# neuripss2020/kccotgan

Measured on AMD Instinct MI355X. Metric: sinkhorn_loss_evals_per_sec, higher is better.
Workload: dtype f32; 1 GPU; BASELINE configs[1]: Moving-MNIST shape B=64,T=30,64x64x1, J=8, 100 Sinkhorn iters, compute_sinkhorn_loss fwd+bwd; global_batch=64, parallelism=single GPU, sinkhorn_exact_shortcut=off, launch=hipGraph replay of forward+backward

## Files before the change

kccotgan_amd/csrc/sinkhorn.hip:

```cpp
#include "common.h"
#include <math.h>
#include "options.h"

#pragma clang fp contract(off)

namespace kccot {

constexpr int SK_MAXN = 128;
constexpr int SK_FUSED_MAXPROB = 4;
constexpr int SK_MAXT = 1024;
constexpr float LOG2E = 1.4426950408889634f;
constexpr float LN2 = 0.6931471805599453f;

__device__ __forceinline__ float fast_exp(float x) { return __builtin_amdgcn_exp2f(x * LOG2E); }
__device__ __forceinline__ float fast_log(float x) { return __builtin_amdgcn_logf(x) * LN2; }

#ifdef KCCOT_DIAG
#ifndef KCCOT_DIAG_IT
#define KCCOT_DIAG_IT 50
#endif
#define KCCOT_DIAG_SLOTS 32
#define KCCOT_STAMP(SLOT) KCCOT_STAMP_IF(it == KCCOT_DIAG_IT, SLOT)
#define KCCOT_STAMP_IF(COND, SLOT)                                                                \
    do {                                                                                          \
        if (a.diag && (COND)) {                                                                   \
            unsigned long long tt_;                                                               \
            __builtin_amdgcn_sched_barrier(0);                                                    \
            asm volatile("s_memtime %0\n\ts_waitcnt lgkmcnt(0)" : "=s"(tt_)::"memory");          \
            __builtin_amdgcn_sched_barrier(0);                                                    \
            if ((threadIdx.x & 63) == 0) a.diag[(blockIdx.x * 16 + (threadIdx.x >> 6)) * KCCOT_DIAG_SLOTS + (SLOT)] = tt_; \
        }                                                                                         \
    } while (0)
#define KCCOT_STAMP_DRAINED(SLOT)                                                                 \
    do {                                                                                          \
        if (a.diag) asm volatile("s_waitcnt vmcnt(0)" ::: "memory");                              \
        KCCOT_STAMP_IF(true, SLOT);                                                               \
    } while (0)
#else
#define KCCOT_STAMP(SLOT) do {} while (0)
#define KCCOT_STAMP_IF(COND, SLOT) do {} while (0)
#define KCCOT_STAMP_DRAINED(SLOT) do {} while (0)
#endif

struct SinkArgs {
    const float* C;
    int n, L, Lmin, stop_mode;
    float eps, inv_eps, thresh;
    float* u_hist;
    float* v_hist;
    float* cost_out;
    int32_t* nits_out;
    float* pi_out;
    unsigned long long* diag;
    float* loss_out;
    int* ticket;
    int shortcut;
    const float* wa;
    const float* wb;
    int w_div;
};

__device__ __forceinline__ const float* weights_of(const float* wa, const float* wb, int w_div, int p, int n, bool rows) {
    if (w_div == 2) return wa + (int64_t)(p / 3) * n;
    if (w_div) return rows ? (p == 2 ? wb : wa) : (p == 1 ? wa : wb);
    return (rows ? wa : wb) + (int64_t)p * n;
}
__device__ __forceinline__ bool weight_ok(float w) { return w > 0.f && w < INFINITY; }

template <int EPT>
__device__ __forceinline__ void load_other(float (&o)[EPT], const float* arr, int q) {
    if constexpr (EPT >= 4) {
#pragma unroll
        for (int m = 0; m < EPT; m += 4) {
            const float4 v = *reinterpret_cast<const float4*>(arr + q * EPT + m);
            o[m] = v.x; o[m + 1] = v.y; o[m + 2] = v.z; o[m + 3] = v.w;
        }
    } else {
#pragma unroll
        for (int m = 0; m < EPT; ++m) o[m] = arr[q * EPT + m];
    }
}

typedef float f32x2 __attribute__((ext_vector_type(2)));

template <int N>
__device__ __forceinline__ void keep_in_regs(float (&r)[N]) {
    if constexpr (N >= 2) {
#pragma unroll
        for (int m = 0; m < N; m += 2) {
            f32x2 t = {r[m], r[m + 1]};
            asm volatile("" : "+v"(t));
            r[m] = t.x; r[m + 1] = t.y;
        }
    } else {
        asm volatile("" : "+v"(r[0]));
    }
}

template <int EPT, int LPR, bool ROW>
__device__ __forceinline__ float half_step(const float (&c2)[EPT], float self, const float* other, int q, float lw2) {
    float o[EPT];
    load_other<EPT>(o, other, q);
    float y[EPT];
    if constexpr (EPT >= 2) {
#pragma unroll
        for (int m = 0; m < EPT; m += 2) {
            f32x2 cc = {c2[m], c2[m + 1]}, oo = {o[m], o[m + 1]}, ss = {self, self};
            const f32x2 t = ROW ? ((ss - cc) + oo) : ((oo - cc) + ss);
            y[m] = t.x; y[m + 1] = t.y;
        }
    } else {
        y[0] = ROW ? ((self - c2[0]) + o[0]) : ((o[0] - c2[0]) + self);
    }
    float mx = y[0];
#pragma unroll
    for (int m = 1; m < EPT; ++m) mx = fmaxf(mx, y[m]);
    mx = seg_max<LPR>(mx);
    const float shift = (mx > -INFINITY && mx < INFINITY) ? mx : 0.f;
    float e[EPT];
    if constexpr (EPT >= 2) {
        const f32x2 sh = {shift, shift};
#pragma unroll
        for (int m = 0; m < EPT; m += 2) {
            const f32x2 yy = {y[m], y[m + 1]};
            const f32x2 d = yy - sh;
            e[m] = __builtin_amdgcn_exp2f(d.x);
            e[m + 1] = __builtin_amdgcn_exp2f(d.y);
        }
    } else {
        e[0] = __builtin_amdgcn_exp2f(y[0] - shift);
    }
#pragma unroll
    for (int w = 1; w < EPT; w *= 2)
#pragma unroll
        for (int m = 0; m + w < EPT; m += 2 * w) e[m] += e[m + w];
    const float s = seg_sum<LPR>(e[0]);
    const float lse2 = __builtin_amdgcn_logf(s) + shift;
    return (lw2 - lse2) + self;
}

template <int EPT, int LPR>
__device__ __forceinline__ void load_costs(const float* __restrict__ C, int n, int line, int q, float k2,
                                           float (&crow)[EPT], float (&ccol)[EPT]) {
#pragma unroll
    for (int m = 0; m < EPT; ++m) {
        const int idx = q * EPT + m;
        const bool ok = line < n && idx < n;
        crow[m] = ok ? C[(int64_t)line * n + idx] * k2 : INFINITY;
        ccol[m] = ok ? C[(int64_t)idx * n + line] * k2 : INFINITY;
    }
}


__device__ __forceinline__ void shortcut_mismatch(int& bits, float sn, float cur, float p2, float p3, float p4) {
    const unsigned b = __float_as_uint(sn);
    bits |= (b != __float_as_uint(cur) ? 2 : 0) | (b != __float_as_uint(p2) ? 4 : 0) |
           (b != __float_as_uint(p3) ? 8 : 0) | (b != __float_as_uint(p4) ? 16 : 0);
}
__device__ __forceinline__ void shortcut_vote(int bits, bool active, int t, int* mis, int it) {
    if (!active) bits = 0;
    int wb = 0;
#pragma unroll
    for (int pp = 1; pp <= 4; ++pp)
        if (__builtin_amdgcn_ballot_w64((bits >> pp) & 1)) wb |= 1 << pp;
    if ((t & 63) == 0 && wb) atomicOr(&mis[it & 3], wb);
}
__device__ __forceinline__ int shortcut_period(int* mis, int it, int t, int& mprev) {
    const int mcur = mis[it & 3];
    if (t == 0) mis[(it + 2) & 3] = 0;
    int per = 0;
#pragma unroll
    for (int pp = 4; pp >= 1; --pp)
        if (it - 1 >= pp && !((mprev >> pp) & 1)) per = pp;
    mprev = mcur;
    return per;
}
__device__ __forceinline__ int shortcut_resume(int L, int Lmin, int stop_mode) {
    int first_stop = (stop_mode == KCCOT_STOP_INDEX) ? Lmin + 1 : Lmin;
    if (first_stop < 1) first_stop = 1;
    return (L < first_stop ? L : first_stop) - 1;
}
__device__ __forceinline__ void fill_history_rows(float* hu, float* hv, int NS, int n, int t, int nits, int K1, int per) {
    const int lo = nits - per + 1;
    for (int e = t; e < (K1 - nits) * n; e += blockDim.x) {
        const int k = nits + 1 + e / n, i = e % n;
        const int src = lo + (k - lo) % per;
        hu[k * NS + i] = hu[src * NS + i];
        hv[k * NS + i] = hv[src * NS + i];
    }
}

template <int EPT>
__device__ __forceinline__ float cost_partial(const float (&crow)[EPT], const float (&craw)[EPT], float ui, const float* v,
                                              int n, int q, bool active) {
    float ov[EPT];
    load_other<EPT>(ov, v, q);
    float part = 0.f;
#pragma unroll
    for (int m = 0; m < EPT; ++m) {
        const float pi = __builtin_amdgcn_exp2f((ui - crow[m]) + ov[m]);
        const float sum = part + pi * craw[m];
        part = (active && q * EPT + m < n) ? sum : part;
    }
    return part;
}
template <int EPT, bool ROW>
__device__ __forceinline__ void load_costs_raw(const float* C, int n, int line, int q, float k2, float (&c2)[EPT],
                                               float (&craw)[EPT]) {
#pragma unroll
    for (int m = 0; m < EPT; ++m) {
        const int idx = q * EPT + m;
        const bool ok = line < n && idx < n;
        craw[m] = ok ? C[ROW ? (int64_t)line * n + idx : (int64_t)idx * n + line] : 0.f;
        c2[m] = ok ? craw[m] * k2 : INFINITY;
    }
}
template <int EPT, bool ROW>
__device__ __forceinline__ void load_costs_raw(const float* C, int n, int line, int q, float k2, float (&c2)[EPT]) {
    float craw[EPT];
    load_costs_raw<EPT, ROW>(C, n, line, q, k2, c2, craw);
}

__device__ __forceinline__ float cost_of_waves(const float* red, int nw) {
    float v[16];
#pragma unroll
    for (int w = 0; w < 16; ++w) v[w] = red[w];
    float r = 0.f;
#pragma unroll
    for (int w = 0; w < 16; ++w) r = w < nw ? r + v[w] : r;
    return r;
}

template <int NPROB>
__device__ __forceinline__ void publish_cost(float* const& cost_out, int32_t* const& nits_out, float* const& loss_out,
                                             int* const& ticket, int p, float cost, int nits, int computed, const float* w,
                                             bool combine) {
    __hip_atomic_store(cost_out + p, cost, __ATOMIC_RELAXED, __HIP_MEMORY_SCOPE_AGENT);
    nits_out[p] = nits;
    nits_out[gridDim.x + p] = computed;
    if (!combine) return;
    asm volatile("s_waitcnt vmcnt(0)" ::: "memory");
    const int tk = __hip_atomic_fetch_add(ticket, 1, __ATOMIC_RELAXED, __HIP_MEMORY_SCOPE_AGENT);
    if (tk == (int)gridDim.x - 1) {
        float c[NPROB];
        if constexpr (NPROB == 3) {
#pragma unroll
            for (int pp = 0; pp < 3; ++pp) c[pp] = __hip_atomic_load(cost_out + pp, __ATOMIC_RELAXED, __HIP_MEMORY_SCOPE_AGENT);
        } else {
            float o[3];
#pragma unroll
            for (int k = 0; k < 3; ++k)
                o[k] = __hip_atomic_load(cost_out + ((p + 1 + k) & 3), __ATOMIC_RELAXED, __HIP_MEMORY_SCOPE_AGENT);
#pragma unroll
            for (int pp = 0; pp < 4; ++pp) {
                const int k = (pp - p - 1) & 3;
                c[pp] = k == 0 ? o[0] : k == 1 ? o[1] : k == 2 ? o[2] : cost;
            }
        }
        float l = w[0] * c[0];
#pragma unroll
        for (int pp = 1; pp < NPROB; ++pp) l += w[pp] * c[pp];
        loss_out[0] = l;
        __hip_atomic_store(ticket, 0, __ATOMIC_RELAXED, __HIP_MEMORY_SCOPE_AGENT);
    }
}

template <bool ROW>
__device__ __forceinline__ void final_cost_adjoint(float c2, float self, float other, bool ok, float g, float& d, float& ss) {
    const float cc = ok ? c2 : 0.f;
    const float pv = ok ? __builtin_amdgcn_exp2f(ROW ? ((self - cc) + other) : ((other - cc) + self)) : 0.f;
    d = ROW ? g * pv * (1.f - cc * LN2) : 0.f;
    ss += pv * cc;
}

template <int EPT>
__device__ __forceinline__ void park_dc_cols(float* tile, const float (&dcol)[EPT], int n, int line, int q, bool active) {
    if (active) {
#pragma unroll
        for (int m = 0; m < EPT; ++m) {
            const int idx = q * EPT + m;
            if (idx < n) tile[idx * (n + 1) + line] = dcol[m];
        }
    }
}
template <int EPT>
__device__ __forceinline__ void take_dc_cols(const float* tile, float (&drow)[EPT], int n, int line, int q, bool active) {
#pragma unroll
    for (int m = 0; m < EPT; ++m) {
        const int idx = q * EPT + m;
        drow[m] += tile[(active && idx < n) ? line * (n + 1) + idx : 0];
    }
}
template <int EPT>
__device__ __forceinline__ void store_dc_rows(float* dC, const float (&drow)[EPT], int n, int line, int q, bool active) {
    if (active) {
#pragma unroll
        for (int m = 0; m < EPT; ++m) {
            const int idx = q * EPT + m;
            if (idx < n) dC[(int64_t)line * n + idx] = drow[m];
        }
    }
}

template <int EPT, int LPR, bool SHORTCUT, bool WEIGHTED>
__device__ __forceinline__ void sinkhorn_fwd_body(const SinkArgs& a) {
    __shared__ __attribute__((aligned(16))) float u_s[SK_MAXN + 16 * 16];
    __shared__ __attribute__((aligned(16))) float v_s[SK_MAXN + 16 * 16];
    __shared__ float red[16];
    const int p = blockIdx.x, n = a.n;
    const int t = threadIdx.x, line = t / LPR, q = t % LPR;
    const bool active = line < n;
    int pc = p;
    if constexpr (WEIGHTED) { if (a.w_div == 2) pc = p % 3; }
    const float* C = a.C + (int64_t)pc * n * n;
    const float k2 = a.inv_eps * LOG2E;

    float crow[EPT], ccol[EPT];
    load_costs<EPT, LPR>(C, n, line, q, k2, crow, ccol);
    for (int i = t; i < SK_MAXN + 16 * 16; i += blockDim.x) { u_s[i] = 0.f; v_s[i] = 0.f; }
    __syncthreads();

    const float lw2 = __builtin_amdgcn_logf(1.0f / (float)n);
    float lwu = lw2, lwv = lw2;
    bool bad = false;
    if constexpr (WEIGHTED) {
        const float wu = active ? weights_of(a.wa, a.wb, a.w_div, p, n, true)[line] : 1.f;
        const float wv = active ? weights_of(a.wa, a.wb, a.w_div, p, n, false)[line] : 1.f;
        bad = __syncthreads_or(!(weight_ok(wu) && weight_ok(wv)));
        lwu = __builtin_amdgcn_logf(wu);
        lwv = __builtin_amdgcn_logf(wv);
    }
    const int Lrun = (WEIGHTED && bad) ? 0 : a.L;
    const float err_scale = a.eps * LN2;

    __shared__ float ring_u[4][SK_MAXN], ring_v[4][SK_MAXN];
    __shared__ int mis[4];
    if (SHORTCUT) {
        if (t < 4) mis[t] = 0;
        __syncthreads();
    }
    bool detect = SHORTCUT;
    int computed = 0;
    int mprev = ~0;
    float pu2 = 0.f, pu3 = 0.f, pu4 = 0.f, pv2 = 0.f, pv3 = 0.f, pv4 = 0.f;

    int nits = 0;
    float ui = 0.f, vj = 0.f;
    for (int it = 0; it < Lrun; ++it) {
        KCCOT_STAMP(0);
        const float un = half_step<EPT, LPR, true>(crow, ui, v_s, q, lwu);
        KCCOT_STAMP(1);
        const float du = (active && q == 0) ? fabsf(un - ui) : 0.f;
        int bits = 0;
        if (SHORTCUT && detect) {
            shortcut_mismatch(bits, un, ui, pu2, pu3, pu4);
            pu4 = pu3; pu3 = pu2; pu2 = ui;
        }
        ui = un;
        if (active && q == 0) {
            u_s[line] = un;
            if (a.u_hist) a.u_hist[((int64_t)p * a.L + it) * n + line] = un;
            if (SHORTCUT && detect) ring_u[it & 3][line] = un;
        }
        KCCOT_STAMP(2);
        lds_barrier();
        KCCOT_STAMP(3);
        const float vn = half_step<EPT, LPR, false>(ccol, vj, u_s, q, lwv);
        KCCOT_STAMP(4);
        if (SHORTCUT && detect) {
            shortcut_mismatch(bits, vn, vj, pv2, pv3, pv4);
            pv4 = pv3; pv3 = pv2; pv2 = vj;
            shortcut_vote(bits, active, t, mis, it);
        }
        vj = vn;
        if (active && q == 0) {
            v_s[line] = vn;
            if (a.v_hist) a.v_hist[((int64_t)p * a.L + it) * n + line] = vn;
            if (SHORTCUT && detect) ring_v[it & 3][line] = vn;
        }
        KCCOT_STAMP(5);
        lds_barrier();
        KCCOT_STAMP(6);
        nits = it + 1;
        ++computed;
        const bool reached = (a.stop_mode == KCCOT_STOP_INDEX) ? (it >= a.Lmin) : (nits >= a.Lmin);
        if (reached && it + 1 < a.L) {
            const float err = block_sum(du, red) * err_scale;
            if (a.thresh > err) break;
        }
        if (SHORTCUT && detect) {
            const int per = shortcut_period(mis, it, t, mprev);
            KCCOT_STAMP(7);
            if (per) {
                detect = false;
                const int K1 = shortcut_resume(a.L, a.Lmin, a.stop_mode);
                if (K1 > nits) {
                    const int lo = nits - per + 1;
                    if (a.u_hist) {
                        for (int e = t; e < (K1 - nits) * n; e += blockDim.x) {
                            const int k = nits + 1 + e / n, i = e % n;
                            const int slot = (lo + (k - lo) % per - 1) & 3;
                            a.u_hist[((int64_t)p * a.L + (k - 1)) * n + i] = ring_u[slot][i];
                            a.v_hist[((int64_t)p * a.L + (k - 1)) * n + i] = ring_v[slot][i];
                        }
                    }
                    const int slot = (lo + (K1 - lo) % per - 1) & 3;
                    if (t < n) { u_s[t] = ring_u[slot][t]; v_s[t] = ring_v[slot][t]; }
                    __syncthreads();
                    ui = u_s[active ? line : 0];
                    vj = v_s[active ? line : 0];
                    nits = K1;
                    it = K1 - 1;
                }
            }
        }
    }

    float part = 0.f;
    if (active) {
#pragma unroll
        for (int m = 0; m < EPT; ++m) {
            const int idx = q * EPT + m;
            if (idx < n) {
                float pi = __builtin_amdgcn_exp2f((ui - crow[m]) + v_s[idx]);
                if (WEIGHTED && bad) pi = NAN;
                part += pi * C[(int64_t)line * n + idx];
                if (a.pi_out) a.pi_out[(int64_t)p * n * n + (int64_t)line * n + idx] = pi;
            }
        }
    }
    float cost = block_sum(part, red);
    if (WEIGHTED && bad) { cost = NAN; nits = -1; }
    if (t == 0) {
        const float w[3] = {2.0f, -1.0f, -1.0f};
        publish_cost<3>(a.cost_out, a.nits_out, a.loss_out, a.ticket, p, cost, nits, computed, w, a.loss_out != nullptr);
    }
}

template <int EPT, int LPR>
__global__ __launch_bounds__(SK_MAXT) void sinkhorn_fwd_reg(SinkArgs a) { sinkhorn_fwd_body<EPT, LPR, true, false>(a); }
template <int EPT, int LPR>
__global__ __launch_bounds__(SK_MAXT) void sinkhorn_fwd_reg_full(SinkArgs a) { sinkhorn_fwd_body<EPT, LPR, false, false>(a); }
template <int EPT, int LPR>
__global__ __launch_bounds__(SK_MAXT) void sinkhorn_fwd_reg_w(SinkArgs a) { sinkhorn_fwd_body<EPT, LPR, true, true>(a); }
template <int EPT, int LPR>
__global__ __launch_bounds__(SK_MAXT) void sinkhorn_fwd_reg_full_w(SinkArgs a) { sinkhorn_fwd_body<EPT, LPR, false, true>(a); }

struct SinkBwdArgs {
    const float* C;
    const float* u_hist;
    const float* v_hist;
    const int32_t* nits;
    const float* gcost;
    float* dC;
    int n, L;
    float eps, inv_eps;
    int div_weights;
    const float* wa;
    const float* wb;
    int w_div;
    float* da;
    float* db;
};

template <int EPT, int LPR, bool WEIGHTED, bool DW = false>
__device__ __forceinline__ void sinkhorn_bwd_body(const SinkBwdArgs& a) {
    static_assert(WEIGHTED || !DW, "the weight gradient belongs to the weighted sweep");
    constexpr int PADN = SK_MAXN + 16 * 16;
    __shared__ __attribute__((aligned(16))) float Ua[WEIGHTED ? 2 : 1][WEIGHTED ? PADN : 4];
    __shared__ __attribute__((aligned(16))) float Va[WEIGHTED ? 2 : 1][WEIGHTED ? PADN : 4];
    __shared__ float lab[WEIGHTED ? 2 : 1][WEIGHTED ? SK_MAXN : 1];
    __shared__ __attribute__((aligned(16))) float U[2][PADN];
    __shared__ __attribute__((aligned(16))) float V[2][PADN];
    __shared__ __attribute__((aligned(16))) float gu[PADN];
    __shared__ __attribute__((aligned(16))) float gv[PADN];
    __shared__ double sab[DW ? 2 : 1][DW ? SK_MAXN : 1];
    __shared__ float gvf[DW ? SK_MAXN : 1];
    __shared__ double mode[DW ? 2 : 1];
    const int p = blockIdx.x, n = a.n;
    const int t = threadIdx.x, line = t / LPR, q = t % LPR;
    const bool active = line < n;
    int pc = p;
    if constexpr (WEIGHTED) { if (a.w_div == 2) pc = p % 3; }
    const float* C = a.C + (int64_t)pc * n * n;
    const float k2 = a.inv_eps * LOG2E;
    const float g = a.div_weights ? (p == 0 ? 2.0f : -1.0f) * a.gcost[0] : a.gcost[p];
    const int nits = a.nits[p];
    const float* uh = a.u_hist + (int64_t)p * a.L * n;
    const float* vh = a.v_hist + (int64_t)p * a.L * n;
    if constexpr (WEIGHTED) {
        if (nits < 0) {
            if (active) {
#pragma unroll
                for (int m = 0; m < EPT; ++m) {
                    const int idx = q * EPT + m;
                    if (idx < n) a.dC[(int64_t)p * n * n + (int64_t)line * n + idx] = NAN;
                }
                if constexpr (DW) {
                    if (q == 0) { a.da[(int64_t)p * n + line] = NAN; a.db[(int64_t)p * n + line] = NAN; }
                }
            }
            return;
        }
        if (t < n) {
            lab[0][t] = __builtin_amdgcn_logf(weights_of(a.wa, a.wb, a.w_div, p, n, true)[t]);
            lab[1][t] = __builtin_amdgcn_logf(weights_of(a.wa, a.wb, a.w_div, p, n, false)[t]);
        }
    }

    float crow[EPT], ccol[EPT], drow[EPT], dcol[EPT];
    load_costs<EPT, LPR>(C, n, line, q, k2, crow, ccol);
#pragma unroll
    for (int m = 0; m < EPT; ++m) { drow[m] = 0.f; dcol[m] = 0.f; }
    for (int i = t; i < PADN; i += blockDim.x) {
        U[0][i] = U[1][i] = V[0][i] = V[1][i] = 0.f;
        gu[i] = gv[i] = 0.f;
        if constexpr (WEIGHTED) Ua[0][i] = Ua[1][i] = Va[0][i] = Va[1][i] = 0.f;
    }
    if constexpr (DW) { if (t < SK_MAXN) sab[0][t] = sab[1][t] = 0.0; }
    __syncthreads();
    auto hist_u = [&](int it, int i) { return it >= 1 ? uh[(int64_t)(it - 1) * n + i] : 0.f; };
    auto hist_v = [&](int it, int i) { return it >= 1 ? vh[(int64_t)(it - 1) * n + i] : 0.f; };
    if (t < n) {
        U[nits & 1][t] = hist_u(nits, t);
        V[nits & 1][t] = hist_v(nits, t);
        V[(nits - 1) & 1][t] = hist_v(nits - 1, t);
        if constexpr (WEIGHTED) {
            Ua[nits & 1][t] = hist_u(nits, t) - lab[0][t];
            Va[nits & 1][t] = hist_v(nits, t) - lab[1][t];
            Va[(nits - 1) & 1][t] = hist_v(nits - 1, t) - lab[1][t];
        }
    }
    float nu = (t < n) ? hist_u(nits - 1, t) : 0.f;
    float nv = (t < n) ? hist_v(nits - 2, t) : 0.f;
    __syncthreads();

    const int lsafe = active ? line : 0;
    {
        const float* Uc = U[nits & 1];
        const float* Vc = V[nits & 1];
        const float ui = Uc[lsafe], vj = Vc[lsafe];
        float ov[EPT], ou[EPT];
        load_other<EPT>(ov, Vc, q);
        load_other<EPT>(ou, Uc, q);
        float su = 0.f, sv = 0.f;
#pragma unroll
        for (int m = 0; m < EPT; ++m) {
            const bool ok = active && (q * EPT + m) < n;
            const float cr = ok ? crow[m] : 0.f, cc = ok ? ccol[m] : 0.f;
            const float pr = ok ? __builtin_amdgcn_exp2f((ui - cr) + ov[m]) : 0.f;
            drow[m] = g * pr * (1.f - cr * LN2);
            su += pr * cr;
            const float pc = ok ? __builtin_amdgcn_exp2f((ou[m] - cc) + vj) : 0.f;
            sv += pc * cc;
        }
        su = seg_sum<LPR>(su);
        sv = seg_sum<LPR>(sv);
        if (active && q == 0) {
            const float gvn = g * sv * LN2;
            gu[line] = g * su * LN2; gv[line] = gvn;
            if constexpr (DW) gvf[line] = nits > 0 ? gvn : 0.f;
        }
    }
    const float lw2 = __builtin_amdgcn_logf(1.0f / (float)n);
    __syncthreads();

    for (int it = nits; it >= 1; --it) {
        const float* Uc = U[it & 1];
        const float* Vc = V[it & 1];
        const float* Vp = V[(it - 1) & 1];
        {
            const float ui = WEIGHTED ? Uc[lsafe] : Uc[lsafe] - lw2;
            float ov[EPT], og[EPT];
            load_other<EPT>(ov, WEIGHTED ? Va[it & 1] : Vc, q);
            load_other<EPT>(og, gv, q);
            float s = 0.f;
#pragma unroll
            for (int m = 0; m < EPT; ++m) {
                const float w = __builtin_amdgcn_exp2f((ui - crow[m]) + ov[m]) * og[m];
                drow[m] += w;
                s += w;
            }
            s = seg_sum<LPR>(s);
            if (active && q == 0) {
                const float gun = (it == nits ? gu[line] : 0.f) - s;
                gu[line] = gun;
                if constexpr (DW) sab[0][line] += (double)gun;
            }
        }
        lds_barrier();
        if (t < n) {
            U[(it - 1) & 1][t] = nu;
            V[it & 1][t] = nv;
            if constexpr (WEIGHTED) { Ua[(it - 1) & 1][t] = nu - lab[0][t]; Va[it & 1][t] = nv - lab[1][t]; }
            nu = hist_u(it - 2, t);
            nv = hist_v(it - 3, t);
        }
        {
            const float vj = WEIGHTED ? Vp[lsafe] : Vp[lsafe] - lw2;
            float ou[EPT], og[EPT];
            load_other<EPT>(ou, WEIGHTED ? Ua[it & 1] : Uc, q);
            load_other<EPT>(og, gu, q);
            float r = 0.f;
#pragma unroll
            for (int m = 0; m < EPT; ++m) {
                const float w = __builtin_amdgcn_exp2f((ou[m] - ccol[m]) + vj) * og[m];
                dcol[m] += w;
                r += w;
            }
            r = seg_sum<LPR>(r);
            if (active && q == 0) {
                gv[line] = -r;
                if constexpr (DW) { if (it > 1) sab[1][line] += (double)(-r); }
            }
        }
        lds_barrier();
    }

    if constexpr (DW) {
        const float* pa = weights_of(a.wa, a.wb, a.w_div, p, n, true);
        const float* pb = weights_of(a.wa, a.wb, a.w_div, p, n, false);
        if (t < 64) {
            double ea = 0.0, eb = 0.0, ta = 0.0, tb = 0.0;
            for (int i = t; i < n; i += 64) { ea += sab[0][i]; eb += sab[1][i]; ta += (double)pa[i]; tb += (double)pb[i]; }
            ea = wave_sum_d(ea); eb = wave_sum_d(eb); ta = wave_sum_d(ta); tb = wave_sum_d(tb);
            if (t == 0) { mode[0] = ea / ta; mode[1] = eb / tb; }
        }
        __syncthreads();
        if (active && q == 0) {
            const SinkBwdArgs* ka = (const SinkBwdArgs*)__builtin_amdgcn_kernarg_segment_ptr();
            const double wa = (double)pa[line], wb = (double)pb[line];
            ka->da[(int64_t)p * n + line] = (float)((double)a.eps * (sab[0][line] - mode[0] * wa) / wa);
            ka->db[(int64_t)p * n + line] = (float)((double)a.eps * (((double)gvf[line] + sab[1][line]) - mode[1] * wb) / wb);
        }
    }
    float* dC = a.dC + (int64_t)p * n * n;
    if (active) {
#pragma unroll
        for (int m = 0; m < EPT; ++m) {
            const int idx = q * EPT + m;
            if (idx < n) dC[(int64_t)line * n + idx] = drow[m];
        }
    }
    __threadfence_block();
    __syncthreads();
    if (active) {
#pragma unroll
        for (int m = 0; m < EPT; ++m) {
            const int idx = q * EPT + m;
            if (idx < n) dC[(int64_t)idx * n + line] += dcol[m];
        }
    }
}

template <int EPT, int LPR>
__global__ __launch_bounds__(SK_MAXT) void sinkhorn_bwd_reg(SinkBwdArgs a) { sinkhorn_bwd_body<EPT, LPR, false>(a); }
template <int EPT, int LPR>
__global__ __launch_bounds__(SK_MAXT) void sinkhorn_bwd_reg_w(SinkBwdArgs a) { sinkhorn_bwd_body<EPT, LPR, true>(a); }
template <int EPT, int LPR>
__global__ __launch_bounds__(SK_MAXT) void sinkhorn_bwd_reg_dw(SinkBwdArgs a) { sinkhorn_bwd_body<EPT, LPR, true, true>(a); }

struct SinkFusedArgs {
    const float* C;
    int n, L, Lmin;
    float eps, inv_eps, thresh;
    float* cost_out;
    int32_t* nits_out;
    float* loss_out;
    int* ticket;
    float* dC;
    float w[SK_FUSED_MAXPROB];
    unsigned long long* diag;
};

template <int EPT, int LPR, bool SHORTCUT, int NPROB>
__global__ __launch_bounds__(LPR * SK_MAXN < SK_MAXT ? LPR * SK_MAXN : SK_MAXT) void sinkhorn_fused_reg(SinkFusedArgs a) {
    static_assert(NPROB == 3 || NPROB == 4, "three (compute_sinkhorn_loss) or four (mixed, two minibatches) problems");
    constexpr int NS = EPT * LPR;
    extern __shared__ __attribute__((aligned(16))) float hist[];
    __shared__ __attribute__((aligned(16))) float gu[SK_MAXN + 16 * 16];
    __shared__ __attribute__((aligned(16))) float gv[SK_MAXN + 16 * 16];
    __shared__ __attribute__((aligned(16))) float red[16];
    __shared__ int mis[4];
    const int p = blockIdx.x, n = a.n, L = a.L;
    const int t = threadIdx.x, line = t / LPR, q = t % LPR;
    const bool active = line < n;
    const float* C = a.C + (int64_t)p * n * n;
    const float k2 = a.inv_eps * LOG2E;
    float* hu = hist;
    float* hv = hist + (size_t)(L + 1) * NS;

    KCCOT_STAMP_IF(true, 16);
    const int nw = blockDim.x >> 6;
    const float g = a.w[p];
    float crow[EPT], ccol[EPT], craw[EPT];
    load_costs_raw<EPT, true>(C, n, line, q, k2, crow, craw);
    load_costs_raw<EPT, false>(C, n, line, q, k2, ccol);
    for (int i = t; i < NS; i += blockDim.x) { hu[i] = 0.f; hv[i] = 0.f; }
    if (NS > n) {
        const int padw = NS - n;
        for (int e = t; e < L * padw; e += blockDim.x) {
            const int k = 1 + e / padw, i = n + e % padw;
            hu[k * NS + i] = 0.f; hv[k * NS + i] = 0.f;
        }
    }
    for (int i = t; i < SK_MAXN + 16 * 16; i += blockDim.x) { gu[i] = 0.f; gv[i] = 0.f; }
    if (t < 4) mis[t] = 0;
    __syncthreads();

    const float lw2 = __builtin_amdgcn_logf(1.0f / (float)n);
    const float err_scale = a.eps * LN2;
    bool detect = SHORTCUT;
    int computed = 0;
    int mprev = ~0;
    float pu2 = 0.f, pu3 = 0.f, pu4 = 0.f, pv2 = 0.f, pv3 = 0.f, pv4 = 0.f;
    int nits = 0;
    float ui = 0.f, vj = 0.f;
    KCCOT_STAMP_IF(true, 11);
    for (int it = 0; it < L; ++it) {
        KCCOT_STAMP(9);
        const float un = half_step<EPT, LPR, true>(crow, ui, hv + it * NS, q, lw2);
        const float du = (active && q == 0) ? fabsf(un - ui) : 0.f;
        int bits = 0;
        if (SHORTCUT && detect) {
            shortcut_mismatch(bits, un, ui, pu2, pu3, pu4);
            pu4 = pu3; pu3 = pu2; pu2 = ui;
        }
        ui = un;
        if (active && q == 0) hu[(it + 1) * NS + line] = un;
        lds_barrier();
        const float vn = half_step<EPT, LPR, false>(ccol, vj, hu + (it + 1) * NS, q, lw2);
        if (SHORTCUT && detect) {
            shortcut_mismatch(bits, vn, vj, pv2, pv3, pv4);
            pv4 = pv3; pv3 = pv2; pv2 = vj;
            shortcut_vote(bits, active, t, mis, it);
        }
        vj = vn;
        if (active && q == 0) hv[(it + 1) * NS + line] = vn;
        lds_barrier();
        KCCOT_STAMP(10);
        nits = it + 1;
        ++computed;
        if (nits >= a.Lmin && it + 1 < L) {
            const float err = block_sum(du, red) * err_scale;
            if (a.thresh > err) break;
        }
        if (SHORTCUT && detect) {
            const int per = shortcut_period(mis, it, t, mprev);
            if (per) {
                detect = false;
                const int K1 = shortcut_resume(L, a.Lmin, KCCOT_STOP_COUNT);
                if (K1 > nits) {
                    fill_history_rows(hu, hv, NS, n, t, nits, K1, per);
                    __syncthreads();
                    ui = hu[K1 * NS + (active ? line : 0)];
                    vj = hv[K1 * NS + (active ? line : 0)];
                    nits = K1;
                    it = K1 - 1;
                }
            }
        }
    }

    KCCOT_STAMP_IF(true, 12);
    const float* Vn = hv + nits * NS;
    const float* Un = hu + nits * NS;
    const float psum = wave_sum(cost_partial<EPT>(crow, craw, ui, Vn, n, q, active));
    KCCOT_STAMP_IF(true, 17);

    const int lsafe = active ? line : 0;
    float drow[EPT], dcol[EPT];
    {
        const float uf = Un[lsafe], vf = Vn[lsafe];
        float ov[EPT], ou[EPT];
        load_other<EPT>(ov, Vn, q);
        load_other<EPT>(ou, Un, q);
        float su = 0.f, sv = 0.f;
#pragma unroll
        for (int m = 0; m < EPT; ++m) {
            const bool ok = active && (q * EPT + m) < n;
            final_cost_adjoint<true>(crow[m], uf, ov[m], ok, g, drow[m], su);
            final_cost_adjoint<false>(ccol[m], vf, ou[m], ok, g, dcol[m], sv);
        }
        su = seg_sum<LPR>(su);
        sv = seg_sum<LPR>(sv);
        if (active && q == 0) { gu[line] = g * su * LN2; gv[line] = g * sv * LN2; }
    }
    KCCOT_STAMP_IF(true, 20);
    lds_barrier();
    float qa[EPT], pb[EPT];
    auto plan_a = [&](int it) {
        const float uu = hu[it * NS + lsafe] - lw2;
        float ov[EPT];
        load_other<EPT>(ov, hv + it * NS, q);
#pragma unroll
        for (int m = 0; m < EPT; ++m) qa[m] = __builtin_amdgcn_exp2f((uu - crow[m]) + ov[m]);
    };
    auto plan_b = [&](int it) {
        const float vv = hv[(it - 1) * NS + lsafe] - lw2;
        float ou[EPT];
        load_other<EPT>(ou, hu + it * NS, q);
#pragma unroll
        for (int m = 0; m < EPT; ++m) pb[m] = __builtin_amdgcn_exp2f((ou[m] - ccol[m]) + vv);
    };
    KCCOT_STAMP_IF(true, 13);
    if (nits >= 1) plan_a(nits);
    for (int it = nits; it >= 1; --it) {
        {
            KCCOT_STAMP(0);
            float og[EPT];
            load_other<EPT>(og, gv, q);
            plan_b(it);
            __builtin_amdgcn_sched_barrier(0);
            KCCOT_STAMP(1);
            float sa = 0.f;
#pragma unroll
            for (int m = 0; m < EPT; ++m) {
                const float w = qa[m] * og[m];
                drow[m] += w;
                sa += w;
            }
            sa = seg_sum<LPR>(sa);
            KCCOT_STAMP(2);
            if (active && q == 0) gu[line] = (it == nits ? gu[line] : 0.f) - sa;
            KCCOT_STAMP(3);
        }
        lds_barrier();
        {
            KCCOT_STAMP(4);
            float og[EPT];
            load_other<EPT>(og, gu, q);
            if (it > 1) plan_a(it - 1);
            __builtin_amdgcn_sched_barrier(0);
            KCCOT_STAMP(5);
            float r = 0.f;
#pragma unroll
            for (int m = 0; m < EPT; ++m) {
                const float w = pb[m] * og[m];
                dcol[m] += w;
                r += w;
            }
            r = seg_sum<LPR>(r);
            KCCOT_STAMP(6);
            if (active && q == 0) gv[line] = -r;
            KCCOT_STAMP(7);
        }
        lds_barrier();
        KCCOT_STAMP(8);
    }
    KCCOT_STAMP_IF(true, 14);
    float* dC = a.dC + (int64_t)p * n * n;
    park_dc_cols<EPT>(hist, dcol, n, line, q, active);
    if ((t & 63) == 0) red[t >> 6] = psum;
    lds_barrier();
    KCCOT_STAMP_IF(true, 21);
    take_dc_cols<EPT>(hist, drow, n, line, q, active);
    store_dc_rows<EPT>(dC, drow, n, line, q, active);
    if (t == 0) publish_cost<NPROB>(a.cost_out, a.nits_out, a.loss_out, a.ticket, p, cost_of_waves(red, nw), nits, computed, a.w, true);
    KCCOT_STAMP_IF(true, 19);
    KCCOT_STAMP_DRAINED(22);
}

#ifndef KCCOT_SWEEP_PRIO
#define KCCOT_SWEEP_PRIO 1
#endif
#ifndef KCCOT_SWEEP_PRIO_LEVEL
#define KCCOT_SWEEP_PRIO_LEVEL 1
#endif
template <bool ON>
__device__ __forceinline__ void sweep_prio(bool raised) {
    if constexpr (ON) {
        if (raised) __builtin_amdgcn_s_setprio(KCCOT_SWEEP_PRIO_LEVEL); else __builtin_amdgcn_s_setprio(0);
    }
}

template <int EPT, int LPR, bool SHORTCUT, int NPROB, bool COL>
__device__ __forceinline__ void fused_roles_body(const SinkFusedArgs& a, float* hist, float* gu, float* gv, float* red,
                                                 int* mis, const int TR) {
    constexpr int NS = EPT * LPR;
    const int p = blockIdx.x, n = a.n, L = a.L;
    const int t = threadIdx.x, tr = t - (COL ? TR : 0), line = tr / LPR, q = tr % LPR;
    const bool active = line < n;
    const float* C = a.C + (int64_t)p * n * n;
    const float k2 = a.inv_eps * LOG2E;
    float* hu = hist;
    float* hv = hist + (size_t)(L + 1) * NS;
    float* hs = COL ? hv : hu;
    const float* ho = COL ? hu : hv;

    KCCOT_STAMP_IF(true, 16);
    float c2[EPT];
    float craw[EPT];
    const float g = a.w[p];
    load_costs_raw<EPT, !COL>(C, n, line, q, k2, c2, craw);
    for (int i = t; i < NS; i += blockDim.x) { hu[i] = 0.f; hv[i] = 0.f; }
    if (NS > n) {
        const int padw = NS - n;
        for (int e = t; e < L * padw; e += blockDim.x) {
            const int k = 1 + e / padw, i = n + e % padw;
            hu[k * NS + i] = 0.f; hv[k * NS + i] = 0.f;
        }
    }
    for (int i = t; i < SK_MAXN + 16 * 16; i += blockDim.x) { gu[i] = 0.f; gv[i] = 0.f; }
    if (t < 4) mis[t] = 0;
    __syncthreads();

    const float lw2 = __builtin_amdgcn_logf(1.0f / (float)n);
    const float err_scale = a.eps * LN2;
    bool detect = SHORTCUT;
    int computed = 0;
    int mprev = ~0;
    float p2 = 0.f, p3 = 0.f, p4 = 0.f;
    int nits = 0;
    float self = 0.f;
    auto own_half_step = [&](int it, float& du) {
        const float sn = half_step<EPT, LPR, !COL>(c2, self, ho + (COL ? it + 1 : it) * NS, q, lw2);
        du = (active && q == 0) ? fabsf(sn - self) : 0.f;
        if (active && q == 0) hs[(it + 1) * NS + line] = sn;
        if (SHORTCUT && detect) {
            int bits = 0;
            shortcut_mismatch(bits, sn, self, p2, p3, p4);
            p4 = p3; p3 = p2; p2 = self;
            shortcut_vote(bits, active, t, mis, it);
        }
        self = sn;
    };
    KCCOT_STAMP_IF(true, 11);
    for (int it = 0; it < L; ++it) {
        KCCOT_STAMP(9);
        float du = 0.f;
        if constexpr (!COL) own_half_step(it, du);
        lds_barrier();
        if constexpr (COL) { float dv; own_half_step(it, dv); }
        lds_barrier();
        KCCOT_STAMP(10);
        nits = it + 1;
        ++computed;
        if (nits >= a.Lmin && it + 1 < L) {
            const float err = block_sum(du, red) * err_scale;
            if (a.thresh > err) break;
        }
        if (SHORTCUT && detect) {
            const int per = shortcut_period(mis, it, t, mprev);
            if (per) {
                detect = false;
                const int K1 = shortcut_resume(L, a.Lmin, KCCOT_STOP_COUNT);
                if (K1 > nits) {
                    fill_history_rows(hu, hv, NS, n, t, nits, K1, per);
                    __syncthreads();
                    self = hs[K1 * NS + (active ? line : 0)];
                    nits = K1;
                    it = K1 - 1;
                }
            }
        }
    }

    KCCOT_STAMP_IF(true, 12);
    const float* Vn = hv + nits * NS;
    const float* Un = hu + nits * NS;
    float psum = 0.f;
    if constexpr (!COL) psum = wave_sum(cost_partial<EPT>(c2, craw, self, Vn, n, q, active));
    KCCOT_STAMP_IF(true, 17);

    const int lsafe = active ? line : 0;
    float d[EPT];
    {
        const float sf = (COL ? Vn : Un)[lsafe];
        float oo[EPT];
        load_other<EPT>(oo, COL ? Un : Vn, q);
        float ss = 0.f;
#pragma unroll
        for (int m = 0; m < EPT; ++m) final_cost_adjoint<!COL>(c2[m], sf, oo[m], active && (q * EPT + m) < n, g, d[m], ss);
        ss = seg_sum<LPR>(ss);
        if (active && q == 0) (COL ? gv : gu)[line] = g * ss * LN2;
    }
    KCCOT_STAMP_IF(true, 20);
    lds_barrier();
    float pl[EPT];
    auto plan = [&](int it) {
        const float sv = hs[(COL ? it - 1 : it) * NS + lsafe] - lw2;
        float oo[EPT];
        load_other<EPT>(oo, ho + it * NS, q);
#pragma unroll
        for (int m = 0; m < EPT; ++m) pl[m] = __builtin_amdgcn_exp2f(COL ? ((oo[m] - c2[m]) + sv) : ((sv - c2[m]) + oo[m]));
    };
    auto chain = [&](int it) {
        float og[EPT];
        load_other<EPT>(og, COL ? gu : gv, q);
        KCCOT_STAMP(COL ? 5 : 1);
        float s = 0.f;
#pragma unroll
        for (int m = 0; m < EPT; ++m) {
            const float w = pl[m] * og[m];
            d[m] += w;
            s += w;
        }
        s = seg_sum<LPR>(s);
        KCCOT_STAMP(COL ? 6 : 2);
        if (active && q == 0) {
            if constexpr (COL) gv[line] = -s;
            else gu[line] = (it == nits ? gu[line] : 0.f) - s;
        }
        KCCOT_STAMP(COL ? 7 : 3);
    };
    KCCOT_STAMP_IF(true, 13);
    if constexpr (!COL) { if (nits >= 1) { plan(nits); keep_in_regs(pl); } }
    if constexpr (COL) sweep_prio<KCCOT_SWEEP_PRIO == 3>(true);
    for (int it = nits; it >= 1; --it) {
        KCCOT_STAMP(0);
        if constexpr (COL) { plan(it); keep_in_regs(pl); KCCOT_STAMP(1); }
        else { sweep_prio<KCCOT_SWEEP_PRIO == 1>(true); chain(it); sweep_prio<KCCOT_SWEEP_PRIO == 1>(false); }
        lds_barrier();
        KCCOT_STAMP(4);
        if constexpr (COL) { sweep_prio<KCCOT_SWEEP_PRIO == 1 || KCCOT_SWEEP_PRIO == 2>(true); chain(it); sweep_prio<KCCOT_SWEEP_PRIO == 1 || KCCOT_SWEEP_PRIO == 2>(false); }
        else { if (it > 1) { plan(it - 1); keep_in_regs(pl); } KCCOT_STAMP(5); }
        lds_barrier();
        KCCOT_STAMP(8);
    }
    if constexpr (COL) sweep_prio<KCCOT_SWEEP_PRIO == 3>(false);
    KCCOT_STAMP_IF(true, 14);
    float* dC = a.dC + (int64_t)p * n * n;
    if constexpr (COL) park_dc_cols<EPT>(hist, d, n, line, q, active);
    if ((t & 63) == 0) red[t >> 6] = psum;
    lds_barrier();
    KCCOT_STAMP_IF(true, 21);
    if constexpr (!COL) {
        take_dc_cols<EPT>(hist, d, n, line, q, active);
        store_dc_rows<EPT>(dC, d, n, line, q, active);
    } else {
        if (tr == 0) publish_cost<NPROB>(a.cost_out, a.nits_out, a.loss_out, a.ticket, p, cost_of_waves(red, TR >> 5), nits, computed, a.w, true);
        KCCOT_STAMP_IF(true, 19);
    }
    KCCOT_STAMP_DRAINED(22);
}

template <int EPT, int LPR, bool SHORTCUT, int NPROB>
__global__ __launch_bounds__(SK_MAXT) void sinkhorn_fused_roles(SinkFusedArgs a) {
    static_assert(NPROB == 3 || NPROB == 4, "three (compute_sinkhorn_loss) or four (mixed, two minibatches) problems");
    extern __shared__ __attribute__((aligned(16))) float hist[];
    __shared__ __attribute__((aligned(16))) float gu[SK_MAXN + 16 * 16];
    __shared__ __attribute__((aligned(16))) float gv[SK_MAXN + 16 * 16];
    __shared__ __attribute__((aligned(16))) float red[16];
    __shared__ int mis[4];
    const int TR = blockDim.x >> 1;
    if (__builtin_amdgcn_readfirstlane((int)threadIdx.x >= TR)) fused_roles_body<EPT, LPR, SHORTCUT, NPROB, true>(a, hist, gu, gv, red, mis, TR);
    else fused_roles_body<EPT, LPR, SHORTCUT, NPROB, false>(a, hist, gu, gv, red, mis, TR);
}

__global__ void mixed_divergence_fwd(const float* __restrict__ cost3, float* __restrict__ loss) {
    if (threadIdx.x == 0) loss[0] = (2.0f * cost3[0] - cost3[1]) - cost3[2];
}
__global__ void mixed_divergence_bwd(const float* __restrict__ gloss, float* __restrict__ gcost3) {
    if (threadIdx.x == 0) {
        const float g = gloss[0];
        gcost3[0] = 2.0f * g; gcost3[1] = -g; gcost3[2] = -g;
    }
}

struct SinkGeom { int lpr, ept, threads; };

static SinkGeom sink_geom(int n, bool forward) {
    SinkGeom g;
    g.lpr = (n <= 32) ? 16 : (n <= 64 ? (forward ? 8 : 16) : 8);
    if (n > 32 && n <= 64) {
        const int v = opt(OPT_SK_LPR);
        if (v == 4 || v == 8 || v == 16) g.lpr = v;
    }
    const int need = (n + g.lpr - 1) / g.lpr;
    g.ept = need <= 1 ? 1 : need <= 2 ? 2 : need <= 4 ? 4 : need <= 8 ? 8 : 16;
    g.threads = (n * g.lpr + 63) / 64 * 64;
    return g;
}

}

namespace kccot {
size_t sinkhorn_gen_workspace_bytes(int nprob, int n);
int launch_sinkhorn_fwd_gen(const float* C, int nprob, int n, float eps, int L, int Lmin, float thresh, int stop_mode,
                            float* u_hist, float* v_hist, float* cost_out, int32_t* nits_out, float* pi_out, void* ws,
                            size_t ws_bytes, hipStream_t st, const float* wa, const float* wb, int w_div);
int launch_sinkhorn_bwd_gen(const float* C, const float* u_hist, const float* v_hist, const int32_t* nits, int nprob, int n,
                            float eps, int L, const float* gcost, float* dC, void* ws, size_t ws_bytes, hipStream_t st,
                            const float* wa, const float* wb, int w_div, float* da, float* db);
}

using namespace kccot;

static int sink_shortcut_enabled() { return opt(OPT_SK_SHORTCUT); }

extern "C" size_t kccot_sinkhorn_workspace_bytes(int nprob, int n) {
    if (nprob <= 0 || n <= SK_MAXN) return 0;
    return sinkhorn_gen_workspace_bytes(nprob, n);
}

#define KCCOT_SK_LAUNCH(KERNEL, E, P, ARGS, GEOM, NPROB, ST) \
    hipLaunchKernelGGL((KERNEL<E, P>), dim3(NPROB), dim3((GEOM).threads), 0, ST, ARGS)

#define KCCOT_SK_DISPATCH(KERNEL, ARGS, GEOM, NPROB, ST)                                       \
    if ((GEOM).lpr == 16) {                                                                    \
        switch ((GEOM).ept) {                                                                  \
            case 1: KCCOT_SK_LAUNCH(KERNEL, 1, 16, ARGS, GEOM, NPROB, ST); break;              \
            case 2: KCCOT_SK_LAUNCH(KERNEL, 2, 16, ARGS, GEOM, NPROB, ST); break;              \
            default: KCCOT_SK_LAUNCH(KERNEL, 4, 16, ARGS, GEOM, NPROB, ST); break;             \
        }                                                                                      \
    } else if ((GEOM).lpr == 4) {                                                              \
        KCCOT_SK_LAUNCH(KERNEL, 16, 4, ARGS, GEOM, NPROB, ST);                                 \
    } else {                                                                                   \
        switch ((GEOM).ept) {                                                                  \
            case 8: KCCOT_SK_LAUNCH(KERNEL, 8, 8, ARGS, GEOM, NPROB, ST); break;               \
            default: KCCOT_SK_LAUNCH(KERNEL, 16, 8, ARGS, GEOM, NPROB, ST); break;             \
        }                                                                                      \
    }

static int sinkhorn_fwd(const float* C, int nprob, int n, float eps, int L, int Lmin, float thresh, int stop_mode,
                        float* u_hist, float* v_hist, float* cost_out, int32_t* nits_out, float* pi_out, void* ws,
                        size_t ws_bytes, kccot_stream_t stream, float* div_loss, int* div_ticket,
                        const float* wa = nullptr, const float* wb = nullptr, int w_div = 0) {
    if (!C || !cost_out || !nits_out) return fail(KCCOT_EINVAL, "sinkhorn_fwd: null pointer");
    if ((wa == nullptr) != (wb == nullptr)) return fail(KCCOT_EINVAL, "sinkhorn_fwd: give both weight vectors or neither");
    if (w_div == 1 && nprob != 3) return fail(KCCOT_EINVAL, "sinkhorn_fwd: the divergence's weights need nprob = 3");
    if (w_div == 2 && nprob % 3) return fail(KCCOT_EINVAL, "sinkhorn_fwd: the conditional mode needs nprob = 3 Q");
    if (nprob <= 0 || n <= 0 || L < 0 || !(eps > 0.f))
        return fail(KCCOT_EINVAL, "sinkhorn_fwd: bad arguments nprob=%d n=%d L=%d eps=%g", nprob, n, L, (double)eps);
    if ((u_hist == nullptr) != (v_hist == nullptr))
        return fail(KCCOT_EINVAL, "sinkhorn_fwd: u_hist and v_hist must be given together");
    if (stop_mode != KCCOT_STOP_COUNT && stop_mode != KCCOT_STOP_INDEX)
        return fail(KCCOT_EINVAL, "sinkhorn_fwd: bad stop_mode %d", stop_mode);
    if (n > SK_MAXN)
        return launch_sinkhorn_fwd_gen(C, nprob, n, eps, L, Lmin, thresh, stop_mode, u_hist, v_hist, cost_out, nits_out,
                                       pi_out, ws, ws_bytes, (hipStream_t)stream, wa, wb, w_div);
    SinkGeom g = sink_geom(n, true);
    SinkArgs a{C, n, L, Lmin, stop_mode, eps, (float)(1.0 / (double)eps), thresh, u_hist, v_hist, cost_out, nits_out, pi_out,
               nullptr, div_loss, div_ticket, sink_shortcut_enabled(), wa, wb, w_div};
#ifdef KCCOT_DIAG
    a.diag = static_cast<unsigned long long*>(ws);
#endif
    hipStream_t st = (hipStream_t)stream;
    if (wa) {
        if (a.shortcut) {
            KCCOT_SK_DISPATCH(sinkhorn_fwd_reg_w, a, g, nprob, st)
        } else {
            KCCOT_SK_DISPATCH(sinkhorn_fwd_reg_full_w, a, g, nprob, st)
        }
        return launch_status("sinkhorn_fwd_reg_w");
    }
    if (a.shortcut) {
        KCCOT_SK_DISPATCH(sinkhorn_fwd_reg, a, g, nprob, st)
    } else {
        KCCOT_SK_DISPATCH(sinkhorn_fwd_reg_full, a, g, nprob, st)
    }
    return launch_status("sinkhorn_fwd_reg");
}

extern "C" int kccot_sinkhorn_fwd_f32(const float* C, int nprob, int n, float eps, int L, int Lmin,
                                      float thresh, int stop_mode, float* u_hist, float* v_hist,
                                      float* cost_out, int32_t* nits_out, float* pi_out, void* ws,
                                      size_t ws_bytes, kccot_stream_t stream) {
    return sinkhorn_fwd(C, nprob, n, eps, L, Lmin, thresh, stop_mode, u_hist, v_hist, cost_out, nits_out, pi_out, ws,
                        ws_bytes, stream, nullptr, nullptr);
}

extern "C" int kccot_sinkhorn_status(const int32_t* nits, int nprob, kccot_stream_t stream) {
    if (!nits || nprob <= 0 || nprob > 4096) return fail(KCCOT_EINVAL, "sinkhorn_status: bad arguments");
    int32_t host[4096];
    hipStream_t st = (hipStream_t)stream;
    if (hipMemcpyAsync(host, nits, sizeof(int32_t) * nprob, hipMemcpyDeviceToHost, st) != hipSuccess ||
        hipStreamSynchronize(st) != hipSuccess)
        return fail(KCCOT_EINVAL, "sinkhorn_status: could not read the iteration counts");
    for (int p = 0; p < nprob; ++p)
        if (host[p] < 0)
            return fail(KCCOT_EABORTED, "sinkhorn: problem %d of %d was aborted -- a workgroup of the multi-CU solver never "
                        "arrived (device shared or partitioned?); set KCCOT_SK_NO_COOP=1 to use the one-workgroup solver", p, nprob);
    return 0;
}

static int sinkhorn_bwd(const float* C, const float* u_hist, const float* v_hist, const int32_t* nits, int nprob, int n,
                        float eps, int L, const float* gcost, float* dC_out, void* ws, size_t ws_bytes,
                        kccot_stream_t stream, int div_weights, const float* wa = nullptr, const float* wb = nullptr,
                        int w_div = 0, float* da = nullptr, float* db = nullptr) {
    if (!C || !u_hist || !v_hist || !nits || !gcost || !dC_out)
        return fail(KCCOT_EINVAL, "sinkhorn_bwd: null pointer");
    if ((da == nullptr) != (db == nullptr) || (da && !wa))
        return fail(KCCOT_EINVAL, "sinkhorn_bwd: da and db are given together, with the weights");
// ... 230 lines not shown
```

Before: 5820 loss-evals/s (fwd+bwd).

## Trim forward Sinkhorn critical path in fused-roles kernel

Measured after the change: 6021 loss-evals/s (fwd+bwd), median of 6. +3.5%, better.

```diff
diff --git a/kccotgan_amd/csrc/sinkhorn.hip b/kccotgan_amd/csrc/sinkhorn.hip
--- a/kccotgan_amd/csrc/sinkhorn.hip
+++ b/kccotgan_amd/csrc/sinkhorn.hip
@@ -97,26 +97,40 @@
     }
 }
 
-template <int EPT, int LPR, bool ROW>
-__device__ __forceinline__ float half_step(const float (&c2)[EPT], float self, const float* other, int q, float lw2) {
-    float o[EPT];
-    load_other<EPT>(o, other, q);
-    float y[EPT];
-    if constexpr (EPT >= 2) {
-#pragma unroll
-        for (int m = 0; m < EPT; m += 2) {
-            f32x2 cc = {c2[m], c2[m + 1]}, oo = {o[m], o[m + 1]}, ss = {self, self};
-            const f32x2 t = ROW ? ((ss - cc) + oo) : ((oo - cc) + ss);
-            y[m] = t.x; y[m + 1] = t.y;
-        }
-    } else {
-        y[0] = ROW ? ((self - c2[0]) + o[0]) : ((o[0] - c2[0]) + self);
-    }
+#ifndef KCCOT_FWD_TRIM
+#define KCCOT_FWD_TRIM 23
+#endif
+
+#define KCCOT_DPP_MAX_STEP(CTRL) "s_nop 1\n\tv_max_f32_dpp %0, %0, %0 " CTRL " row_mask:0xf bank_mask:0xf\n\t"
+template <int LPR>
+__device__ __forceinline__ float seg_max_chain(float v) {
+    if constexpr (LPR >= 16)
+        asm volatile(KCCOT_DPP_MAX_STEP("quad_perm:[1,0,3,2]") KCCOT_DPP_MAX_STEP("quad_perm:[2,3,0,1]")
+                     KCCOT_DPP_MAX_STEP("row_half_mirror") KCCOT_DPP_MAX_STEP("row_mirror") : "+v"(v));
+    else if constexpr (LPR >= 8)
+        asm volatile(KCCOT_DPP_MAX_STEP("quad_perm:[1,0,3,2]") KCCOT_DPP_MAX_STEP("quad_perm:[2,3,0,1]")
+                     KCCOT_DPP_MAX_STEP("row_half_mirror") : "+v"(v));
+    else if constexpr (LPR >= 4)
+        asm volatile(KCCOT_DPP_MAX_STEP("quad_perm:[1,0,3,2]") KCCOT_DPP_MAX_STEP("quad_perm:[2,3,0,1]") : "+v"(v));
+    else if constexpr (LPR >= 2)
+        asm volatile(KCCOT_DPP_MAX_STEP("quad_perm:[1,0,3,2]") : "+v"(v));
+    return v;
+}
+
+typedef __attribute__((address_space(3))) float lds_float;
+__device__ __forceinline__ unsigned lds_address(const float* p) { return (unsigned)(size_t)(const lds_float*)p; }
+__device__ __forceinline__ float* lds_pointer(unsigned a) { return (float*)(lds_float*)(size_t)a; }
+
+struct NoStamp { __device__ __forceinline__ void operator()(int) const {} };
+
+template <int EPT, int LPR, bool PAIRS = false, bool ONE_MAX = false, typename STAMP = NoStamp>
+__device__ __forceinline__ float half_step_lse(const float (&y)[EPT], float self, float lw2, STAMP stamp = STAMP()) {
     float mx = y[0];
 #pragma unroll
     for (int m = 1; m < EPT; ++m) mx = fmaxf(mx, y[m]);
-    mx = seg_max<LPR>(mx);
+    mx = ONE_MAX ? seg_max_chain<LPR>(mx) : seg_max<LPR>(mx);
     const float shift = (mx > -INFINITY && mx < INFINITY) ? mx : 0.f;
+    stamp(0);
     float e[EPT];
     if constexpr (EPT >= 2) {
         const f32x2 sh = {shift, shift};
@@ -130,13 +144,46 @@
     } else {
         e[0] = __builtin_amdgcn_exp2f(y[0] - shift);
     }
-#pragma unroll
-    for (int w = 1; w < EPT; w *= 2)
-#pragma unroll
-        for (int m = 0; m + w < EPT; m += 2 * w) e[m] += e[m + w];
+    if constexpr (PAIRS && EPT >= 4) {
+        constexpr int H = EPT / 2;
+        f32x2 pe[H];
+#pragma unroll
+        for (int k = 0; k < H; ++k) pe[k] = f32x2{e[k], e[k + H]};
+#pragma unroll
+        for (int w = 1; w < H; w *= 2)
+#pragma unroll
+            for (int m = 0; m + w < H; m += 2 * w) pe[m] += pe[m + w];
+        e[0] = pe[0].x + pe[0].y;
+    } else {
+#pragma unroll
+        for (int w = 1; w < EPT; w *= 2)
+#pragma unroll
+            for (int m = 0; m + w < EPT; m += 2 * w) e[m] += e[m + w];
+    }
     const float s = seg_sum<LPR>(e[0]);
+    stamp(1);
     const float lse2 = __builtin_amdgcn_logf(s) + shift;
     return (lw2 - lse2) + self;
+}
+
+template <int EPT, int LPR, bool ROW, bool PAIRS = false, bool ONE_MAX = false, typename STAMP = NoStamp>
+__device__ __forceinline__ float half_step(const float (&c2)[EPT], float self, const float* other, int q, float lw2,
+                                           STAMP stamp = STAMP()) {
+    float o[EPT];
+    load_other<EPT>(o, other, q);
+    stamp(-1);
+    float y[EPT];
+    if constexpr (EPT >= 2) {
+#pragma unroll
+        for (int m = 0; m < EPT; m += 2) {
+            f32x2 cc = {c2[m], c2[m + 1]}, oo = {o[m], o[m + 1]}, ss = {self, self};
+            const f32x2 t = ROW ? ((ss - cc) + oo) : ((oo - cc) + ss);
+            y[m] = t.x; y[m + 1] = t.y;
+        }
+    } else {
+        y[0] = ROW ? ((self - c2[0]) + o[0]) : ((o[0] - c2[0]) + self);
+    }
+    return half_step_lse<EPT, LPR, PAIRS, ONE_MAX>(y, self, lw2, stamp);
 }
 
 template <int EPT, int LPR>
@@ -220,6 +267,8 @@
     float craw[EPT];
     load_costs_raw<EPT, ROW>(C, n, line, q, k2, c2, craw);
 }
+
+__device__ __forceinline__ float canonical_nan(float x) { return x != x ? __uint_as_float(0x7fc00000u) : x; }
 
 __device__ __forceinline__ float cost_of_waves(const float* red, int nw) {
     float v[16];
@@ -297,7 +346,7 @@
 #pragma unroll
         for (int m = 0; m < EPT; ++m) {
             const int idx = q * EPT + m;
-            if (idx < n) dC[(int64_t)line * n + idx] = drow[m];
+            if (idx < n) dC[(int64_t)line * n + idx] = canonical_nan(drow[m]);
         }
     }
 }
@@ -350,7 +399,8 @@
         KCCOT_STAMP(0);
         const float un = half_step<EPT, LPR, true>(crow, ui, v_s, q, lwu);
         KCCOT_STAMP(1);
-        const float du = (active && q == 0) ? fabsf(un - ui) : 0.f;
+        float du = 0.f;
+        if (!(KCCOT_FWD_TRIM & 32) || (((a.stop_mode == KCCOT_STOP_INDEX) ? it >= a.Lmin : it + 1 >= a.Lmin) && it + 1 < a.L)) du = (active && q == 0) ? fabsf(un - ui) : 0.f;
         int bits = 0;
         if (SHORTCUT && detect) {
             shortcut_mismatch(bits, un, ui, pu2, pu3, pu4);
@@ -433,7 +483,7 @@
     if (WEIGHTED && bad) { cost = NAN; nits = -1; }
     if (t == 0) {
         const float w[3] = {2.0f, -1.0f, -1.0f};
-        publish_cost<3>(a.cost_out, a.nits_out, a.loss_out, a.ticket, p, cost, nits, computed, w, a.loss_out != nullptr);
+        publish_cost<3>(a.cost_out, a.nits_out, a.loss_out, a.ticket, p, canonical_nan(cost), nits, computed, w, a.loss_out != nullptr);
     }
 }
 
@@ -648,7 +698,8 @@
 #pragma unroll
         for (int m = 0; m < EPT; ++m) {
             const int idx = q * EPT + m;
-            if (idx < n) dC[(int64_t)idx * n + line] += dcol[m];
+            if constexpr (EPT < 16) { if (idx < n) dC[(int64_t)idx * n + line] = canonical_nan(dC[(int64_t)idx * n + line] + dcol[m]); }
+            else { if (idx < n) dC[(int64_t)idx * n + line] += dcol[m]; }
         }
     }
 }
@@ -720,7 +771,8 @@
     for (int it = 0; it < L; ++it) {
         KCCOT_STAMP(9);
         const float un = half_step<EPT, LPR, true>(crow, ui, hv + it * NS, q, lw2);
-        const float du = (active && q == 0) ? fabsf(un - ui) : 0.f;
+        float du = 0.f;
+        if (!(KCCOT_FWD_TRIM & 32) || (it + 1 >= a.Lmin && it + 1 < L)) du = (active && q == 0) ? fabsf(un - ui) : 0.f;
         int bits = 0;
         if (SHORTCUT && detect) {
             shortcut_mismatch(bits, un, ui, pu2, pu3, pu4);
@@ -856,7 +908,7 @@
     KCCOT_STAMP_IF(true, 21);
     take_dc_cols<EPT>(hist, drow, n, line, q, active);
     store_dc_rows<EPT>(dC, drow, n, line, q, active);
-    if (t == 0) publish_cost<NPROB>(a.cost_out, a.nits_out, a.loss_out, a.ticket, p, cost_of_waves(red, nw), nits, computed, a.w, true);
+    if (t == 0) publish_cost<NPROB>(a.cost_out, a.nits_out, a.loss_out, a.ticket, p, canonical_nan(cost_of_waves(red, nw)), nits, computed, a.w, true);
     KCCOT_STAMP_IF(true, 19);
     KCCOT_STAMP_DRAINED(22);
 }
@@ -913,17 +965,41 @@
     float p2 = 0.f, p3 = 0.f, p4 = 0.f;
     int nits = 0;
     float self = 0.f;
+    constexpr bool RUNNING = (KCCOT_FWD_TRIM & 4) && !SHORTCUT;
+    constexpr bool DU_OFF_CHAIN = (KCCOT_FWD_TRIM & 2) && !SHORTCUT;
+    constexpr bool PAIRS = (KCCOT_FWD_TRIM & 16) && !SHORTCUT;
+    constexpr bool ONE_MAX = (KCCOT_FWD_TRIM & 1) != 0;
+    unsigned rb = lds_address(ho + (COL ? NS : 0) + q * EPT);
+    unsigned wb = lds_address(hs + NS + line);
+    float prev = 0.f;
     auto own_half_step = [&](int it, float& du) {
-        const float sn = half_step<EPT, LPR, !COL>(c2, self, ho + (COL ? it + 1 : it) * NS, q, lw2);
-        du = (active && q == 0) ? fabsf(sn - self) : 0.f;
-        if (active && q == 0) hs[(it + 1) * NS + line] = sn;
+        (void)du;
+        const float* other = RUNNING ? lds_pointer(rb) : ho + (COL ? it + 1 : it) * NS + q * EPT;
+        const float sn = half_step<EPT, LPR, !COL, PAIRS, ONE_MAX>(c2, self, other, 0, lw2, [&](int k) { (void)k; KCCOT_STAMP(24 + k); });
+        if constexpr (!DU_OFF_CHAIN) du = (active && q == 0) ? fabsf(sn - self) : 0.f;
+        if (active && q == 0) {
+            if constexpr (RUNNING) *lds_pointer(wb) = sn;
+            else hs[(it + 1) * NS + line] = sn;
+        }
+        KCCOT_STAMP(26);
         if (SHORTCUT && detect) {
             int bits = 0;
             shortcut_mismatch(bits, sn, self, p2, p3, p4);
             p4 = p3; p3 = p2; p2 = self;
             shortcut_vote(bits, active, t, mis, it);
         }
+        if constexpr (DU_OFF_CHAIN) prev = self;
         self = sn;
+    };
+    auto off_chain = [&](int it, float& du) {
+        if constexpr (RUNNING) asm volatile("" : "+v"(self), "+v"(rb), "+v"(wb));
+        if constexpr (DU_OFF_CHAIN && !COL) {
+            if (it + 1 >= a.Lmin && it + 1 < L) du = (active && q == 0) ? fabsf(self - prev) : 0.f;
+        }
+        if constexpr (RUNNING) {
+            rb += NS * 4; wb += NS * 4;
+            asm volatile("" : "+v"(rb), "+v"(wb));
+        }
     };
     KCCOT_STAMP_IF(true, 11);
     for (int it = 0; it < L; ++it) {
@@ -931,9 +1007,12 @@
         float du = 0.f;
         if constexpr (!COL) own_half_step(it, du);
         lds_barrier();
+        KCCOT_STAMP(27);
         if constexpr (COL) { float dv; own_half_step(it, dv); }
+        else off_chain(it, du);
         lds_barrier();
         KCCOT_STAMP(10);
+        if constexpr (COL) { float dv; off_chain(it, dv); }
         nits = it + 1;
         ++computed;
         if (nits >= a.Lmin && it + 1 < L) {
@@ -1029,7 +1108,7 @@
         take_dc_cols<EPT>(hist, d, n, line, q, active);
         store_dc_rows<EPT>(dC, d, n, line, q, active);
     } else {
-        if (tr == 0) publish_cost<NPROB>(a.cost_out, a.nits_out, a.loss_out, a.ticket, p, cost_of_waves(red, TR >> 5), nits, computed, a.w, true);
+        if (tr == 0) publish_cost<NPROB>(a.cost_out, a.nits_out, a.loss_out, a.ticket, p, canonical_nan(cost_of_waves(red, TR >> 5)), nits, computed, a.w, true);
         KCCOT_STAMP_IF(true, 19);
     }
     KCCOT_STAMP_DRAINED(22);
```
